# jonatasfreitasv/hyperopt

Hardware: AMD Instinct MI355X
Metric: EI candidates scored/sec (50-dim, 10k trials) (higher is better)
Workload: dtype f32

## Files before the change

hyperopt_amd/csrc/tpe_table.hip:

```cpp
#include "tpe_table.hpp"

namespace tpe {
namespace {
constexpr double kRhoLim = 5.8;
#ifndef TPE_TAU_TABLE
#define TPE_TAU_TABLE 17.0
#endif
constexpr double kTauExtra = TPE_TAU_TABLE;
constexpr double kDrawZ = 5.8;
#ifndef TPE_BUILD_BLOCKS
#define TPE_BUILD_BLOCKS 384
#endif
constexpr int kBuildBlocks = TPE_BUILD_BLOCKS;
constexpr int kCoopCells = 4096;

__device__ __forceinline__ double admissible_s(double z) {
  return (-9.0 * z + sqrt(81.0 * z * z + 166.0 * kRhoLim)) / 83.0;
}

constexpr int kPlanStride = 4;

__device__ __forceinline__ void plan_range(const tpe_job& J, const tpe_seg& SB, const tpe_seg& S,
                                           const double* __restrict__ mu,
                                           const double* __restrict__ sigma,
                                           const double* __restrict__ coef64, double* red,
                                           double draw_z, double tau, double& a, double& b,
                                           double& T) {
  a = INFINITY;
  b = -INFINITY;
  for (int k = threadIdx.x; k < SB.n_obs + 1; k += kBS) {
    const double m = mu[SB.comp_off + k], sg = sigma[SB.comp_off + k];
    a = fmin(a, m - draw_z * sg);
    b = fmax(b, m + draw_z * sg);
  }
  a = -block_max<kBS, double>(-a, red);
  b = block_max<kBS, double>(b, red);
  if (J.flags & TPE_F_INJECTED) {
    a = fmax(a, J.bin_lo);
    b = fmin(b, J.bin_hi);
  }
  if (J.flags & TPE_F_LOW) a = fmax(a, J.low);
  if (J.flags & TPE_F_HIGH) b = fmin(b, J.high);
  if (!(isfinite(a) && isfinite(b) && b >= a)) {
    const double c = isfinite(a) ? a : (isfinite(b) ? b : SB.prior_mu);
    a = b = c;
  }
  const double4 cp = ld4(coef64, S.comp_off + S.prior_pos);
  const double far = fmax(fabs(a - cp.x), fabs(b - cp.x)) * cp.y;
  T = cp.z - 0.5 * far * far - (log((double)(S.n_obs + 1)) + tau);
}

__device__ __forceinline__ void plan_comp(const tpe_seg& S, const double* __restrict__ sigma,
                                          const double* __restrict__ coef64, double T, int k,
                                          bool& wide, double& hr, double& lr, double& hk) {
  const double4 c = ld4(coef64, S.comp_off + k);
  const double d = c.z - T;
  const double z = d > 0.0 ? sqrt(2.0 * d) : 0.0;
  hk = d > 0.0 ? admissible_s(z) / c.y : INFINITY;
  wide = is_wide(S, k, c.y);
  const double r = z / c.y * (1.0 + 1e-9) + 1e-12 * fabs(c.x);
  hr = wide ? -INFINITY : c.x + r;
  lr = wide ? INFINITY : c.x - r;
}

__global__ __launch_bounds__(kBS) void k_table_plan1(
    const tpe_job* __restrict__ jobs, const tpe_seg* __restrict__ segs,
    const double* __restrict__ mu, const double* __restrict__ sigma,
    const double* __restrict__ coef64, double* __restrict__ reach_hi,
    double* __restrict__ reach_lo, double* __restrict__ part, tpe_table* __restrict__ tables,
    double draw_z, double tau) {
  __shared__ double red[kBS / kWave];
  __shared__ double scan_d[kBS / kWave];
  const int job = blockIdx.y >> 1, half = blockIdx.y & 1;
  const tpe_job J = jobs[job];
  const tpe_seg SB = segs[J.below];
  const tpe_seg S = segs[half ? J.above : J.below];
  const int nc = S.n_obs + 1;
  if ((int)blockIdx.x * kBS >= nc) return;
  double a, b, T;
  plan_range(J, SB, S, mu, sigma, coef64, red, draw_z, tau, a, b, T);
  const int k = blockIdx.x * kBS + threadIdx.x;
  bool wide = true;
  double hr = -INFINITY, lr = INFINITY, hk = INFINITY;
  if (k < nc) plan_comp(S, sigma, coef64, T, k, wide, hr, lr, hk);
  hr = block_prefix_max(hr, scan_d);
  if (k < nc) reach_hi[S.comp_off + k] = hr;
  const int tend = min(nc, (int)(blockIdx.x + 1) * kBS) - 1;
  const int kr = tend - (int)threadIdx.x;
  bool wr;
  double hr2, lr2 = INFINITY, hk2;
  if (kr >= (int)blockIdx.x * kBS) plan_comp(S, sigma, coef64, T, kr, wr, hr2, lr2, hk2);
  lr2 = -block_prefix_max(-lr2, scan_d);
  if (kr >= (int)blockIdx.x * kBS) reach_lo[S.comp_off + kr] = lr2;
  const double tmax = block_max<kBS, double>(hr, red);
  const double tmin = -block_max<kBS, double>(-lr2, red);
  const double nw = block_sum<kBS, double>((k < nc && wide) ? 1.0 : 0.0, red);
  const double hmin = -block_max<kBS, double>(-hk, red);
  if (threadIdx.x == 0) {
    double* P = part + ((int64_t)blockIdx.y * gridDim.x + blockIdx.x) * kPlanStride;
    P[0] = tmax;
    P[1] = tmin;
    P[2] = nw;
    P[3] = hmin;
    if (blockIdx.x == 0) {
      if (half == 0) {
        tables[job].lo = a;
        tables[job].hi = b;
        tables[job].T_below = T;
      } else {
        tables[job].T_above = T;
      }
    }
  }
}

__global__ __launch_bounds__(kBS) void k_table_plan2(
    const tpe_job* __restrict__ jobs, const tpe_seg* __restrict__ segs,
    const double* __restrict__ mu, const double* __restrict__ sigma,
    const double* __restrict__ coef64, double* __restrict__ reach_hi,
    double* __restrict__ reach_lo, int32_t* __restrict__ wide_idx,
    const double* __restrict__ part, tpe_table* __restrict__ tables) {
  __shared__ double red[kBS / kWave];
  __shared__ int scan_n[kBS / kWave];
  const int job = blockIdx.y >> 1, half = blockIdx.y & 1;
  const tpe_job J = jobs[job];
  const tpe_seg S = segs[half ? J.above : J.below];
  const int nc = S.n_obs + 1;
  const int tiles = (nc + kBS - 1) / kBS;
  const int t = blockIdx.x;
  if (t >= tiles) return;
  const double* P = part + (int64_t)blockIdx.y * gridDim.x * kPlanStride;
  double chi = -INFINITY, clo = INFINITY, woff = 0.0, hmin = INFINITY, nw = 0.0;
  for (int q = threadIdx.x; q < tiles; q += kBS) {
    if (q < t) {
      chi = fmax(chi, P[q * kPlanStride]);
      woff += P[q * kPlanStride + 2];
    }
    if (q > t) clo = fmin(clo, P[q * kPlanStride + 1]);
    hmin = fmin(hmin, P[q * kPlanStride + 3]);
    nw += P[q * kPlanStride + 2];
  }
  chi = block_max<kBS, double>(chi, red);
  clo = -block_max<kBS, double>(-clo, red);
  const int wbase = (int)block_sum<kBS, double>(woff, red);
  hmin = -block_max<kBS, double>(-hmin, red);
  const int ntot = (int)block_sum<kBS, double>(nw, red);
  const int k = t * kBS + threadIdx.x;
  bool wide = false;
  if (k < nc) {
    reach_hi[S.comp_off + k] = fmax(reach_hi[S.comp_off + k], chi);
    reach_lo[S.comp_off + k] = fmin(reach_lo[S.comp_off + k], clo);
    wide = is_wide(S, k, ld4(coef64, S.comp_off + k).y);
  }
  const int incl = block_prefix_sum(wide ? 1 : 0, scan_n);
  if (wide) wide_idx[S.comp_off + wbase + incl - 1] = k;
  if (t == 0 && threadIdx.x == 0) {
    if (half == 0) {
      tables[job].h_below = hmin;
      tables[job].n_wide_below = ntot;
      tables[job].build_items = 0;
      tables[job].build_ab = 0.0f;
      tables[job].eps_cubic = 0.0f;
    } else {
      tables[job].h_above = hmin;
      tables[job].n_wide_above = ntot;
    }
  }
}

template <int CTRL, int M>
__device__ __forceinline__ void fold_stage(double (&w)[16], bool hi) {
#pragma unroll
  for (int j = 0; j < M; ++j) {
    const double keep = hi ? w[2 * j + 1] : w[2 * j], send = hi ? w[2 * j] : w[2 * j + 1];
    w[j] = keep + dpp_d<CTRL>(send);
  }
}
__device__ __forceinline__ int rev4(int p) {
  return ((p & 1) << 3) | ((p & 2) << 1) | ((p & 4) >> 1) | ((p & 8) >> 3);
}

struct Windows {
  int lo_b, end_b, lo_a, end_a;
};
__device__ __forceinline__ Windows cell_windows(const tpe_seg& SB, const tpe_seg& SA,
                                                const double* __restrict__ reach_hi,
                                                const double* __restrict__ reach_lo, double ylo,
                                                double yhi) {
  const int lane = lane_id(), g = lane >> 4, l = lane & 15;
  const tpe_seg& S = g < 2 ? SB : SA;
  const bool gt = g & 1;
  const double* a = (gt ? reach_lo : reach_hi) + S.comp_off;
  const double v = gt ? yhi : ylo;
  int lo = 0, hi = S.n_obs + 1;
  while (__any(lo < hi)) {
    const bool active = lo < hi;
    const int stride = (hi - lo + 15) / 16;
    const int idx = lo + l * stride;
    bool p = true;
    if (active && idx < hi) p = gt ? (a[idx] > v) : (a[idx] >= v);
    const uint32_t m = (uint32_t)(__ballot(p) >> (g * 16)) & 0xFFFFu;
    const int f = m ? __builtin_ctz(m) : 16;
    if (active) {
      if (f == 0) {
        hi = lo;
      } else {
        const int nlo = lo + (f - 1) * stride + 1;
        hi = min(lo + f * stride, hi);
        lo = nlo;
      }
    }
  }
  return Windows{__builtin_amdgcn_readlane(lo, 0), __builtin_amdgcn_readlane(lo, 16),
                 __builtin_amdgcn_readlane(lo, 32), __builtin_amdgcn_readlane(lo, 48)};
}

__device__ __forceinline__ double row_sum9_transposed(const double (&P)[9]) {
  const int lane = lane_id();
  double w[16];
#pragma unroll
  for (int n = 0; n < 16; ++n) w[n] = n < 9 ? P[n] : 0.0;
  fold_stage<kDppMirror, 5>(w, (lane >> 3) & 1);
  w[5] = 0.0;
  fold_stage<kDppHalfMirror, 3>(w, (lane >> 2) & 1);
  w[3] = 0.0;
  fold_stage<kDppXor2, 2>(w, (lane >> 1) & 1);
  fold_stage<kDppXor1, 1>(w, lane & 1);
  return w[0];
}

struct BuildLds {
  int m[kBS / kWave][4];
  double p[kBS / kWave][kWave];
  int bad[kBS / kWave][4];
};
constexpr int kNoScale = -100000;
__device__ __forceinline__ bool build_mix(const tpe_seg& S, const double* __restrict__ coef64,
                                          int k_lo, int k_hi,
                                          const int32_t* __restrict__ wide_idx, int n_wide,
                                          double T, double y0, double h, float* cell, bool store,
                                          int mix, double& m_out, BuildLds& X, bool coop,
                                          int& itm) {
  constexpr int kNW = kBS / kWave;
  const int wv = coop ? (int)threadIdx.x / kWave : 0;
  const int stride = coop ? 16 * kNW : 16;
  const int64_t off = S.comp_off;
  const int nwin = max(0, k_hi - k_lo + 1);
  const int items = nwin + n_wide;
  itm = max(itm, items);
  const int lane = lane_id(), l = lane & 15, row = lane >> 4;
  auto comp = [&](int it) -> int {
    return it < nwin ? k_lo + it : wide_idx[off + (it - nwin)];
  };
  const float hf = (float)h, Tf = (float)T;
  constexpr int kP64 = 4;
  double P[kP64];
  float Q[kP - kP64];
#pragma unroll
  for (int n = 0; n < kP64; ++n) P[n] = 0.0;
#pragma unroll
  for (int n = 0; n < kP - kP64; ++n) Q[n] = 0.0f;
  auto acc = [&](int n, float t) __attribute__((always_inline)) {
    if (n < kP64)
      P[n] += (double)t;
    else
      Q[n - kP64] += t;
  };
  auto rescale = [&](int d) __attribute__((always_inline)) {
#pragma unroll
    for (int n = 0; n < kP64; ++n) P[n] = ldexp(P[n], d);
#pragma unroll
    for (int n = 0; n < kP - kP64; ++n) Q[n] = ldexpf(Q[n], d);
  };
  int sl = kNoScale;
  bool bad = false;
  int it = wv * 16 + l;
  int k = it < items ? comp(it) : 0;
  double4 c = it < items ? ld4(coef64, off + k) : make_double4(0.0, 0.0, 0.0, 0.0);
  for (; it < items; it += stride) {
    const int itn = it + stride;
    const int kn = itn < items ? comp(itn) : 0;
    const double4 cn = itn < items ? ld4(coef64, off + kn) : c;
    const bool skip = it < nwin && is_wide(S, k, c.y);
    const double dy = y0 - c.x;
    const float dyf = (float)dy, inv = (float)c.y;
    const float zn = fmaxf(fabsf(dyf) - hf, 0.0f) * inv;
    const bool inc = !skip && ((float)c.z - 0.5f * zn * zn >= Tf);
    const double zc = dy * c.y;
    const double t2 = (c.z - 0.5 * zc * zc) * kLog2e;
    const bool up = inc && t2 > (double)(sl + 8);
    if (__any(up)) {
      if (up) {
        const int ns = (int)ceil(t2);
        rescale(max(sl - ns, -1100));
        sl = ns;
      }
    }
    const float hi2 = hf * inv * inv;
    const float Af = inc ? -dyf * hi2 : 0.0f, B2 = inc ? -hf * hi2 : 0.0f;
    bad = bad || (9.0f * fabsf(Af) + 32.5f * fabsf(B2) > (float)(kRhoLim * (1.0 + 1e-5)));
    const double xs = t2 - (double)sl, xn = floor(xs);
    const float e = inc ? ldexpf(__builtin_amdgcn_exp2f((float)(xs - xn)), (int)xn) : 0.0f;
    float cm = 0.0f, cc = e;
    acc(0, e);
#pragma unroll
    for (int n = 0; n + 1 < kP; ++n) {
      const float cnx = fmaf(Af, cc, B2 * cm) * (1.0f / (float)(n + 1));
      acc(n + 1, cnx);
      cm = cc;
      cc = cnx;
    }
    k = kn;
    c = cn;
  }
  int sr = row_max_i(sl);
  rescale(max(sl - sr, -1100));
  static_assert(kP == 9, "row_sum9_transposed folds nine terms");
  double Pall[kP];
#pragma unroll
  for (int n = 0; n < kP; ++n) Pall[n] = n < kP64 ? P[n] : (double)Q[n - kP64];
  double tot = row_sum9_transposed(Pall);
  bad = ((__ballot(bad) >> (lane & ~15)) & 0xFFFFull) != 0;
  bool anybad = bad;
  if (coop) {
    if (l == 0) {
      X.bad[wv][row] = bad;
      X.m[wv][row] = sr;
    }
    X.p[wv][lane] = tot;
    __syncthreads();
    int sb = X.m[0][row];
#pragma unroll
    for (int w = 1; w < kNW; ++w) sb = max(sb, X.m[w][row]);
    tot = 0.0;
    anybad = false;
    for (int w = 0; w < kNW; ++w) {
      tot += ldexp(X.p[w][lane], max(X.m[w][row] - sb, -1100));
      anybad = anybad || X.bad[w][row];
    }
    sr = sb;
    __syncthreads();
  }
  const double p0 = __shfl(tot, lane & ~15, kWave);
  int e0 = 0;
  if (p0 > 0.0) {
    (void)frexp(p0, &e0);
    e0 -= 1;
    tot = ldexp(tot, -e0);
  }
  const int n = rev4(l);
  if (store && wv == 0 && n < kP) {
    if (n < kP32)
      cell[2 * n + mix] = (float)tot;
    else
      reinterpret_cast<_Float16*>(cell + 2 * kP32)[2 * (n - kP32) + mix] = (_Float16)(float)tot;
  }
  m_out = (p0 > 0.0) ? (double)(sr + e0) * kLn2 : -INFINITY;
  return anybad;
}

constexpr double kFitTol = 1.0e-6;
constexpr int kScoreLanes = 8;
constexpr int kScoreCellsPerBlock = kBS / kScoreLanes;
#ifndef TPE_SCORE_BLOCKS
#define TPE_SCORE_BLOCKS 160
#endif
constexpr int kScoreBlocks = TPE_SCORE_BLOCKS;
constexpr double kUFit = 1.0501;
constexpr int kLogD = 7;
constexpr int kLogM = 12;
constexpr double kU32 = 0x1.0p-24;
constexpr double kAbMax = 0.6768;

__host__ __device__ inline double mix_eps(int items, bool coop, double ab) {
  const double u = kU32, ud = 0x1.0p-53;
  const int stride = coop ? 64 : 16;
  const int K = (items + stride - 1) / stride + 5 + (coop ? 5 : 0);
  const double E1 = exp(ab), E2 = E1 * E1;
  return 4.4e-7
         + exp(-kTauExtra) * 1.0001
         + 0.6932 * u + 1e-13
         + 0x1.0p-22
         + 5.5 * u * ab
         + 4.0 * u * ab * E2
         + u * E2
         + (K + 1) * u * 0.0198 * 1.0001
         + 1.5e-7 + 0x1.0p-25 * 4.2 * E1
         + (K + 8) * 2.0 * ud * E2;
}

__device__ __forceinline__ void cell_coefs(const float* cell, int mix, double (&p)[kP]) {
  const _Float16* tail = reinterpret_cast<const _Float16*>(cell + 2 * kP32);
#pragma unroll
  for (int n = 0; n < kP32; ++n) p[n] = (double)cell[2 * n + mix];
#pragma unroll
  for (int n = kP32; n < kP; ++n) p[n] = (double)(float)tail[2 * (n - kP32) + mix];
}

__device__ __forceinline__ bool log_taylor(const double (&p)[kP], double c, double r, double& lnT0,
                                           double (&l)[kLogD + 1], double& rem) {
  double T[kP];
#pragma unroll
  for (int n = 0; n < kP; ++n) T[n] = p[n];
#pragma unroll
  for (int i = 0; i < kP - 1; ++i)
#pragma unroll
    for (int j = kP - 2; j >= i; --j) T[j] = fma(c, T[j + 1], T[j]);
  if (!(T[0] > 0.0) || !isfinite(T[0])) return false;
  lnT0 = log(T[0]);
  const double inv0 = 1.0 / T[0];
  double a[kP];
  a[0] = 1.0;
#pragma unroll
  for (int k = 1; k < kP; ++k) a[k] = T[k] * inv0;
  l[0] = 0.0;
#pragma unroll
  for (int k = 1; k <= kLogD; ++k) {
    double s = 0.0;
#pragma unroll
    for (int j = 1; j < k; ++j) s = fma((double)j * l[j], a[k - j], s);
    l[k] = a[k] - s * (1.0 / (double)k);
  }
  float aa[kP], m[kLogM + 1];
  float w4 = 0.0f, rr = 1.0f;
  const float r4 = (float)(4.0 * r);
#pragma unroll
  for (int k = 1; k < kP; ++k) {
    aa[k] = (float)fabs(a[k]);
    rr *= r4;
    w4 = fmaf(aa[k], rr, w4);
  }
  w4 *= 1.001f;
  if (!(w4 <= 0.5f)) return false;
  float tail = 0.0f, rk = 1.0f, jm[kLogM + 1];
  const float rf = (float)r;
#pragma unroll
  for (int k = 1; k <= kLogM; ++k) {
    float s = 0.0f;
#pragma unroll
    for (int j = 1; j < k; ++j)
      if (k - j < kP) s = fmaf(jm[j], aa[k - j], s);
    const float mk = fmaf(s, 1.0f / (float)k, k < kP ? aa[k] : 0.0f);
    m[k] = mk;
    jm[k] = (float)k * mk;
    rk *= rf;
    if (k > kLogD) tail = fmaf(mk, rk, tail);
  }
  rem = (double)tail * 1.001 + 0.6931471805599453 * ldexp(1.0, -2 * (kLogM + 1)) / 0.75;
  return true;
}

#ifndef TPE_TSCORE_WPE
#define TPE_TSCORE_WPE 4
#endif
__global__ __launch_bounds__(kBS) __attribute__((amdgpu_waves_per_eu(TPE_TSCORE_WPE))) void k_table_score(const tpe_job* __restrict__ jobs,
                                                     tpe_table* __restrict__ tables,
                                                     float* __restrict__ cells,
                                                     unsigned long long* __restrict__ stats) {
  __shared__ float fred[kBS / kWave];
  const tpe_job J = jobs[blockIdx.y];
  const tpe_table Tb = tables[blockIdx.y];
  const int nb = Tb.nb;
  if (blockIdx.x == 0 && threadIdx.x == 0) {
    tables[blockIdx.y].build_ab = (float)kAbMax;
    tables[blockIdx.y].eps_mix =
        (float)(mix_eps(Tb.build_items, nb <= kCoopCells, kAbMax) * (1.0 + 1e-6));
  }
  char* region = reinterpret_cast<char*>(cells) + J.tbl_off * kSlotB;
  float4* outs = const_cast<float4*>(score_cells_of(region, J.tbl_cap));
  const int sub = threadIdx.x / kScoreLanes, l = threadIdx.x % kScoreLanes;
  const int gbase = lane_id() & ~(kScoreLanes - 1);
  constexpr double kU = (double)kULim;
  const double nd0 = kU * 0.92387953251128674, nd1 = kU * 0.38268343236508978, nd2 = -nd1,
               nd3 = -nd0;
  const double un = l == 0 ? nd0 : l == 1 ? nd1 : l == 2 ? nd2 : nd3;
  const double i10 = 1.0 / (nd1 - nd0), i21 = 1.0 / (nd2 - nd1), i32 = 1.0 / (nd3 - nd2),
               i20 = 1.0 / (nd2 - nd0), i31 = 1.0 / (nd3 - nd1), i30 = 1.0 / (nd3 - nd0);
  const float uf = (float)un;
  const float du_lg = lgmm_du(J, Tb);
  constexpr double r = kUFit / kScoreLanes;
  const double cI = -kUFit + (2 * l + 1) * r;
  float slope = 0.0f, epsc = 0.0f;
  for (int64_t c = (int64_t)blockIdx.x * kScoreCellsPerBlock + sub; c < nb;
       c += (int64_t)gridDim.x * kScoreCellsPerBlock) {
    const float* cell = reinterpret_cast<const float*>(region) + c * kCellF;
    const double off = (double)cell[15];
    const _Float16* tail = reinterpret_cast<const _Float16*>(cell + 2 * kP32);
    float pb = 0.0f, pa = 0.0f;
#pragma unroll
    for (int n = kP - 1; n >= kP32; --n) {
      pb = fmaf(pb, uf, (float)tail[2 * (n - kP32)]);
      pa = fmaf(pa, uf, (float)tail[2 * (n - kP32) + 1]);
    }
#pragma unroll
    for (int n = kP32 - 1; n >= 0; --n) {
      pb = fmaf(pb, uf, cell[2 * n]);
      pa = fmaf(pa, uf, cell[2 * n + 1]);
    }
    const bool ok_pt = (pb > 0.0f) && (pa > 0.0f) && isfinite(pb) && isfinite(pa);
    int e = 0;
    const float mt = ok_pt ? frexpf(pb / pa, &e) : 1.0f;
    const double f = off + kLn2 * ((double)e + (double)__builtin_amdgcn_logf(mt));
    const double f0 = __shfl(f, gbase + 0, kWave), f1 = __shfl(f, gbase + 1, kWave),
                 f2 = __shfl(f, gbase + 2, kWave), f3 = __shfl(f, gbase + 3, kWave);
    const bool nodes_ok = ((__ballot(!ok_pt) >> gbase) & 0xFull) == 0;
    const double d01 = (f1 - f0) * i10, d12 = (f2 - f1) * i21, d23 = (f3 - f2) * i32;
    const double d012 = (d12 - d01) * i20, d123 = (d23 - d12) * i31;
    const double d0123 = (d123 - d012) * i30;
    const double c3 = d0123;
    const double c2 = d012 - d0123 * (nd0 + nd1 + nd2);
    const double c1 = d01 - d012 * (nd0 + nd1) + d0123 * (nd0 * nd1 + nd0 * nd2 + nd1 * nd2);
    const double c0 = f0 - d01 * nd0 + d012 * nd0 * nd1 - d0123 * nd0 * nd1 * nd2;
    const float4 q = make_float4((float)c0, (float)c1, (float)c2, (float)c3);
    const double q0 = q.x, q1 = q.y, q2 = q.z, q3 = q.w;
    bool fail = !nodes_ok || !(off == off) || !isfinite(q0) || !isfinite(q1) || !isfinite(q2) ||
                !isfinite(q3);
    double bound = INFINITY;
    if (!fail) {
      double pbv[kP], pav[kP], lb[kLogD + 1], la[kLogD + 1], lnb = 0.0, lna = 0.0, rb = 0.0,
             ra = 0.0;
      cell_coefs(cell, 0, pbv);
      cell_coefs(cell, 1, pav);
      const bool okb = log_taylor(pbv, cI, r, lnb, lb, rb);
      const bool oka = log_taylor(pav, cI, r, lna, la, ra);
      if (okb && oka) {
        const double qc = ((q3 * cI + q2) * cI + q1) * cI + q0;
        const double qk[4] = {qc, (3.0 * q3 * cI + 2.0 * q2) * cI + q1, 3.0 * q3 * cI + q2, q3};
        const double E0 = off + lnb - lna - qc;
        double sum = fabs(E0), rk = 1.0;
#pragma unroll
        for (int k = 1; k <= kLogD; ++k) {
          rk *= r;
          const double Ek = lb[k] - la[k] - (k < 4 ? qk[k] : 0.0);
          sum = fma(fabs(Ek), rk, sum);
        }
        const double slack = 1e-13 * (1.0 + fabs(off) + fabs(lnb) + fabs(lna) + fabs(qc));
        bound = sum + rb + ra + slack;
      }
    }
    float bmax = (float)(bound * (1.0 + 1e-6));
#pragma unroll
    for (int o = 1; o < kScoreLanes; o <<= 1) bmax = fmaxf(bmax, __shfl_xor(bmax, o, kWave));
    if (!(bmax == bmax)) bmax = INFINITY;
    fail = fail || !(bmax <= (float)kFitTol);
    const bool bad = ((__ballot(fail) >> gbase) & ((1ull << kScoreLanes) - 1)) != 0;
    if (l == 0) {
      outs[c] = bad ? make_float4(__int_as_float(0x7FC00000), 0.0f, 0.0f, 0.0f) : q;
      if (bad && stats) atomicAdd(stats + 2, 1ull);
      if (!bad) {
        const float sl = fabsf(q.y) + 2.11f * fabsf(q.z) + 3.31f * fabsf(q.w);
        slope = fmaxf(slope, sl);
        const float ev = 0x1.0p-21f * (1.0501f * fabsf(q.y) + 1.1028f * fabsf(q.z) +
                                        1.1581f * fabsf(q.w));
        const float ec = bmax + ev + (4.5f * 0x1.0p-24f + du_lg) * sl +
                         0x1.0p-24f * 1.0001f * (float)fabs(off);
        epsc = fmaxf(epsc, ec * 1.0001f);
      }
    }
  }
  slope = block_max<kBS, float>(slope, fred);
  epsc = block_max<kBS, float>(epsc, fred);
  if (threadIdx.x == 0 && slope > 0.0f)
    atomicMax(reinterpret_cast<unsigned int*>(&tables[blockIdx.y].slope), __float_as_uint(slope));
  if (threadIdx.x == 0 && epsc > 0.0f)
    atomicMax(reinterpret_cast<unsigned int*>(&tables[blockIdx.y].eps_cubic),
              __float_as_uint(epsc));
}

#ifndef TPE_BUILD_WPE
#define TPE_BUILD_WPE 1
#endif
__global__ __launch_bounds__(kBS) __attribute__((amdgpu_waves_per_eu(TPE_BUILD_WPE))) void k_table_build(
    const tpe_job* __restrict__ jobs, const tpe_seg* __restrict__ segs,
    const double* __restrict__ sigma, const double* __restrict__ coef64,
    const double* __restrict__ reach_hi, const double* __restrict__ reach_lo,
    const int32_t* __restrict__ wide_idx, tpe_table* __restrict__ tables,
    float* __restrict__ cells, unsigned long long* __restrict__ stats) {
  const tpe_job J = jobs[blockIdx.y];
  const tpe_table Tb = tables[blockIdx.y];
  const tpe_seg SB = segs[J.below], SA = segs[J.above];
  static_assert(kRefineCells <= kCoopCells, "a refined grid builds cooperatively");
  const Grid g = grid_of(Tb, J.tbl_cap, SB.n_obs + SA.n_obs + 2);
  if (blockIdx.x == 0 && threadIdx.x == 0) {
    tpe_table* W = tables + blockIdx.y;
    W->origin = g.origin;
    W->h = g.h;
    W->inv_h = (float)(1.0 / g.h);
    W->inv_w = (float)(0.5 / g.h);
    W->nb = g.nb;
    W->slope = 0.0f;
  }
  const int wid = threadIdx.x / kWave, row = lane_id() >> 4;
  float* region = cells + J.tbl_off * (kSlotB / 4);
  __shared__ BuildLds X;
  const bool coop = g.nb <= kCoopCells;
  const int64_t q0 = coop ? blockIdx.x : (int64_t)blockIdx.x * (kBS / kWave) + wid;
  const int64_t qs = coop ? gridDim.x : (int64_t)gridDim.x * (kBS / kWave);
  int itm = 0;
  for (int64_t q = q0; 4 * q < g.nb; q += qs) {
    const int c0 = (int)(4 * q), c1 = min(c0 + 3, g.nb - 1);
    const int c = c0 + row;
    const bool mine = c < g.nb;
    const double y0 = (double)cell_centre((float)g.origin, (float)g.h, min(c, c1));
    const double ylo = (double)cell_centre((float)g.origin, (float)g.h, c0) - g.h;
    const double yhi = (double)cell_centre((float)g.origin, (float)g.h, c1) + g.h;
    float* out = region + (int64_t)min(c, c1) * kCellF;
    double mb, ma;
    const Windows w = cell_windows(SB, SA, reach_hi, reach_lo, ylo, yhi);
    const bool bb = build_mix(SB, coef64, w.lo_b, w.end_b - 1, wide_idx, Tb.n_wide_below,
                              Tb.T_below, y0, g.h, out, mine, 0, mb, X, coop, itm);
    const bool ba = build_mix(SA, coef64, w.lo_a, w.end_a - 1, wide_idx, Tb.n_wide_above,
                              Tb.T_above, y0, g.h, out, mine, 1, ma, X, coop, itm);
    if ((!coop || wid == 0) && (lane_id() & 15) == 0 && mine) {
      out[15] = (bb || ba) ? __int_as_float(0x7FC00000) : (float)(mb - ma);
      float* mp = region + (int64_t)J.tbl_cap * kCellF + 2 * c;
      mp[0] = (float)mb;
      mp[1] = (float)ma;
      if ((bb || ba) && stats) atomicAdd(stats + 1, 1ull);
    }
  }
  if (lane_id() == 0 && itm > 0) atomicMax(&tables[blockIdx.y].build_items, itm);
}
}

void launch_table_plan(const tpe_job* jobs, int n_jobs, const tpe_seg* segs, const double* mu,
                       const double* sigma, const double* coef64, int max_comp, double* reach_hi,
                       double* reach_lo, int32_t* wide_idx, double* scratch, tpe_table* tables,
                       double draw_z, double tau, hipStream_t st) {
  const dim3 pg((max_comp + kBS - 1) / kBS, 2 * n_jobs);
  hipLaunchKernelGGL(k_table_plan1, pg, dim3(kBS), 0, st, jobs, segs, mu, sigma, coef64, reach_hi,
                     reach_lo, scratch, tables, draw_z, tau);
  hipLaunchKernelGGL(k_table_plan2, pg, dim3(kBS), 0, st, jobs, segs, mu, sigma, coef64, reach_hi,
                     reach_lo, wide_idx, scratch, tables);
}
}

using namespace tpe;

extern "C" int64_t tpe_table_scratch_bytes(int n_jobs, int max_comp) {
  if (n_jobs < 0 || max_comp < 0) return -1;
  const int64_t tiles = std::max(1, (max_comp + kBS - 1) / kBS);
  return 8 * (int64_t)kPlanStride * tiles * 2 * std::max(n_jobs, 1);
}

extern "C" int tpe_table_build(const tpe_job* jobs, const tpe_job* host_jobs, int n_jobs,
                               const tpe_seg* segs, const double* mu, const double* sigma,
                               const double* coef64, int max_comp, double* reach_hi,
                               double* reach_lo, int32_t* wide_idx, double* scratch,
                               tpe_table* tables, float* cells, uint64_t* stats, void* stream) {
  bool inj = false;
  if (!check_gmm_jobs("tpe_table_build", host_jobs, n_jobs, 65535, kJobTable, &inj))
    return TPE_E_ARG;
  if (n_jobs == 0) return TPE_OK;
  if (!jobs || !segs || !mu || !sigma || !coef64 || !reach_hi || !reach_lo || !wide_idx ||
      !scratch || !tables || !cells) {
    set_error("tpe_table_build: null pointer");
    return TPE_E_ARG;
  }
  if (max_comp < 1 || n_jobs > 32767) {
    set_error("tpe_table_build: max_comp=%d n_jobs=%d", max_comp, n_jobs);
    return TPE_E_ARG;
  }
  hipStream_t st = (hipStream_t)stream;
  launch_table_plan(jobs, n_jobs, segs, mu, sigma, coef64, max_comp, reach_hi, reach_lo, wide_idx,
                    scratch, tables, kDrawZ, kTauExtra, st);
  hipLaunchKernelGGL(k_table_build, dim3(kBuildBlocks, n_jobs), dim3(kBS), 0, st, jobs, segs,
                     sigma, coef64, reach_hi, reach_lo, wide_idx, tables, cells,
                     (unsigned long long*)stats);
  int64_t cap = 1;
  for (int i = 0; i < n_jobs; ++i) cap = std::max(cap, host_jobs[i].tbl_cap);
  const int64_t sblocks =
      std::min<int64_t>(kScoreBlocks, (cap + kScoreCellsPerBlock - 1) / kScoreCellsPerBlock);
  hipLaunchKernelGGL(k_table_score, dim3((unsigned)sblocks, n_jobs), dim3(kBS), 0, st, jobs, tables,
                     cells, (unsigned long long*)stats);
  return check_launch("tpe_table_build");
}
```

Measured before the change: 185.9 billion.

## Tighten table-build inner loop: scalar uniforms, double-buffered loads, cheaper scale tracking

Rewrites the per-item body of the mixture table build as an inlined lambda and restructures the loop into a manually double-buffered ping-pong of coefficient loads, using empty asm barriers to pin load arrival. Grid and threshold values are forced into scalar registers via readfirstlane. The scale level is kept as a double, the wide-component test is inlined, the bad flag becomes a running max, and the first series term is peeled. The aim is to cut VGPR pressure and per-item conversions in the build kernel, at the cost of inline asm and a preprocessor-selected old path kept for diagnostics.

```diff
diff --git a/hyperopt_amd/csrc/tpe_table.hip b/hyperopt_amd/csrc/tpe_table.hip
--- a/hyperopt_amd/csrc/tpe_table.hip
+++ b/hyperopt_amd/csrc/tpe_table.hip
@@ -229,6 +229,18 @@
   return w[0];
 }
 
+__device__ __forceinline__ float uniform_f(float v) {
+  float r;
+  asm("s_nop 1\n\tv_readfirstlane_b32 %0, %1\n\ts_nop 1" : "=s"(r) : "v"(v));
+  return r;
+}
+__device__ __forceinline__ double uniform_d(double v) {
+  const uint64_t u = __builtin_bit_cast(uint64_t, v);
+  const uint32_t lo = (uint32_t)__builtin_amdgcn_readfirstlane((int)(uint32_t)u);
+  const uint32_t hi = (uint32_t)__builtin_amdgcn_readfirstlane((int)(uint32_t)(u >> 32));
+  return __builtin_bit_cast(double, ((uint64_t)hi << 32) | lo);
+}
+
 struct BuildLds {
   int m[kBS / kWave][4];
   double p[kBS / kWave][kWave];
@@ -238,11 +250,11 @@
 __device__ __forceinline__ bool build_mix(const tpe_seg& S, const double* __restrict__ coef64,
                                           int k_lo, int k_hi,
                                           const int32_t* __restrict__ wide_idx, int n_wide,
-                                          double T, double y0, double h, float* cell, bool store,
+                                          float Tf, double y0, float hf, float* cell, bool store,
                                           int mix, double& m_out, BuildLds& X, bool coop,
                                           int& itm) {
   constexpr int kNW = kBS / kWave;
-  const int wv = coop ? (int)threadIdx.x / kWave : 0;
+  const int wv = coop ? __builtin_amdgcn_readfirstlane((int)threadIdx.x / kWave) : 0;
   const int stride = coop ? 16 * kNW : 16;
   const int64_t off = S.comp_off;
   const int nwin = max(0, k_hi - k_lo + 1);
@@ -252,7 +264,6 @@
   auto comp = [&](int it) -> int {
     return it < nwin ? k_lo + it : wide_idx[off + (it - nwin)];
   };
-  const float hf = (float)h, Tf = (float)T;
   constexpr int kP64 = 4;
   double P[kP64];
   float Q[kP - kP64];
@@ -273,46 +284,93 @@
     for (int n = 0; n < kP - kP64; ++n) Q[n] = ldexpf(Q[n], d);
   };
   int sl = kNoScale;
-  bool bad = false;
-  int it = wv * 16 + l;
-  int k = it < items ? comp(it) : 0;
-  double4 c = it < items ? ld4(coef64, off + k) : make_double4(0.0, 0.0, 0.0, 0.0);
-  for (; it < items; it += stride) {
-    const int itn = it + stride;
-    const int kn = itn < items ? comp(itn) : 0;
-    const double4 cn = itn < items ? ld4(coef64, off + kn) : c;
-    const bool skip = it < nwin && is_wide(S, k, c.y);
+  float rho = 0.0f;
+#ifdef TPE_DIAG_BUILD_COPY_LOOP
+#define TPE_SL_D (double)sl
+#define TPE_SL8_D (double)(sl + 8)
+#else
+  double sld = (double)kNoScale, sld8 = (double)(kNoScale + 8);
+#define TPE_SL_D sld
+#define TPE_SL8_D sld8
+#endif
+  const int it_prior = S.prior_pos - k_lo;
+  const double inv_wide = uniform_d(4.0 / S.prior_sigma);
+  auto item = [&](int it, const double4& c) __attribute__((always_inline)) {
+    const bool skip = it < nwin && (it == it_prior || c.y <= inv_wide);
     const double dy = y0 - c.x;
     const float dyf = (float)dy, inv = (float)c.y;
     const float zn = fmaxf(fabsf(dyf) - hf, 0.0f) * inv;
     const bool inc = !skip && ((float)c.z - 0.5f * zn * zn >= Tf);
     const double zc = dy * c.y;
     const double t2 = (c.z - 0.5 * zc * zc) * kLog2e;
-    const bool up = inc && t2 > (double)(sl + 8);
+    const bool up = inc && t2 > TPE_SL8_D;
     if (__any(up)) {
       if (up) {
         const int ns = (int)ceil(t2);
+#ifdef TPE_DIAG_BUILD_COPY_LOOP
         rescale(max(sl - ns, -1100));
         sl = ns;
+#else
+        rescale(max((int)sld - ns, -1100));
+        sld = (double)ns;
+        sld8 = (double)(ns + 8);
+#endif
       }
     }
     const float hi2 = hf * inv * inv;
     const float Af = inc ? -dyf * hi2 : 0.0f, B2 = inc ? -hf * hi2 : 0.0f;
-    bad = bad || (9.0f * fabsf(Af) + 32.5f * fabsf(B2) > (float)(kRhoLim * (1.0 + 1e-5)));
-    const double xs = t2 - (double)sl, xn = floor(xs);
+    rho = fmaxf(rho, 9.0f * fabsf(Af) + 32.5f * fabsf(B2));
+    const double xs = t2 - TPE_SL_D, xn = floor(xs);
     const float e = inc ? ldexpf(__builtin_amdgcn_exp2f((float)(xs - xn)), (int)xn) : 0.0f;
+    acc(0, e);
+#ifdef TPE_DIAG_BUILD_COPY_LOOP
     float cm = 0.0f, cc = e;
-    acc(0, e);
 #pragma unroll
     for (int n = 0; n + 1 < kP; ++n) {
+#else
+    float cm = e, cc = Af * e;
+    acc(1, cc);
+#pragma unroll
+    for (int n = 1; n + 1 < kP; ++n) {
+#endif
       const float cnx = fmaf(Af, cc, B2 * cm) * (1.0f / (float)(n + 1));
       acc(n + 1, cnx);
       cm = cc;
       cc = cnx;
     }
-    k = kn;
+  };
+#undef TPE_SL_D
+#undef TPE_SL8_D
+  int it = wv * 16 + l;
+#ifdef TPE_DIAG_BUILD_COPY_LOOP
+  double4 c = it < items ? ld4(coef64, off + comp(it)) : make_double4(0.0, 0.0, 0.0, 0.0);
+  for (; it < items; it += stride) {
+    const int itn = it + stride;
+    const double4 cn = itn < items ? ld4(coef64, off + comp(itn)) : c;
+    item(it, c);
     c = cn;
   }
+#else
+  auto arrive = [](double4& c) __attribute__((always_inline)) {
+    asm volatile("" : "+v"(c.x), "+v"(c.y), "+v"(c.z));
+  };
+  double4 ca = make_double4(0.0, 0.0, 0.0, 0.0), cb = ca;
+  if (it < items) ca = ld4(coef64, off + comp(it));
+  arrive(ca);
+  while (it < items) {
+    int itn = it + stride;
+    if (itn < items) cb = ld4(coef64, off + comp(itn));
+    item(it, ca);
+    arrive(cb);
+    if (itn >= items) break;
+    it = itn + stride;
+    if (it < items) ca = ld4(coef64, off + comp(it));
+    item(itn, cb);
+    arrive(ca);
+  }
+  sl = (int)sld;
+#endif
+  bool bad = rho > (float)(kRhoLim * (1.0 + 1e-5));
   int sr = row_max_i(sl);
   rescale(max(sl - sr, -1100));
   static_assert(kP == 9, "row_sum9_transposed folds nine terms");
@@ -580,7 +638,11 @@
   const tpe_table Tb = tables[blockIdx.y];
   const tpe_seg SB = segs[J.below], SA = segs[J.above];
   static_assert(kRefineCells <= kCoopCells, "a refined grid builds cooperatively");
-  const Grid g = grid_of(Tb, J.tbl_cap, SB.n_obs + SA.n_obs + 2);
+  Grid g = grid_of(Tb, J.tbl_cap, SB.n_obs + SA.n_obs + 2);
+  g.origin = uniform_d(g.origin);
+  g.h = uniform_d(g.h);
+  const float hf = uniform_f((float)g.h);
+  const float Tfb = uniform_f((float)Tb.T_below), Tfa = uniform_f((float)Tb.T_above);
   if (blockIdx.x == 0 && threadIdx.x == 0) {
     tpe_table* W = tables + blockIdx.y;
     W->origin = g.origin;
@@ -590,7 +652,7 @@
     W->nb = g.nb;
     W->slope = 0.0f;
   }
-  const int wid = threadIdx.x / kWave, row = lane_id() >> 4;
+  const int wid = __builtin_amdgcn_readfirstlane((int)(threadIdx.x / kWave)), row = lane_id() >> 4;
   float* region = cells + J.tbl_off * (kSlotB / 4);
   __shared__ BuildLds X;
   const bool coop = g.nb <= kCoopCells;
@@ -608,9 +670,9 @@
     double mb, ma;
     const Windows w = cell_windows(SB, SA, reach_hi, reach_lo, ylo, yhi);
     const bool bb = build_mix(SB, coef64, w.lo_b, w.end_b - 1, wide_idx, Tb.n_wide_below,
-                              Tb.T_below, y0, g.h, out, mine, 0, mb, X, coop, itm);
+                              Tfb, y0, hf, out, mine, 0, mb, X, coop, itm);
     const bool ba = build_mix(SA, coef64, w.lo_a, w.end_a - 1, wide_idx, Tb.n_wide_above,
-                              Tb.T_above, y0, g.h, out, mine, 1, ma, X, coop, itm);
+                              Tfa, y0, hf, out, mine, 1, ma, X, coop, itm);
     if ((!coop || wid == 0) && (lane_id() & 15) == 0 && mine) {
       out[15] = (bb || ba) ? __int_as_float(0x7FC00000) : (float)(mb - ma);
       float* mp = region + (int64_t)J.tbl_cap * kCellF + 2 * c;
```

Result: no change. 186.3 billion (median of 5 runs) (+0.2%).
